# davxy/ark-vrf

Measured on AMD Instinct MI355X. Metric: thin_vrf_batch_verifications_per_sec, higher is better.
Workload: dtype u32x8 (256-bit prime-field Montgomery, integer)

## Files before the change

### ark_vrf_amd/csrc/curves.h

```cpp
#pragma once
#include <type_traits>
#include "fpn.h"
#include "te.h"
#include "fpu_te.h"
#include "fpu_g1.h"

#ifndef AVRF_TE_ACC_WAVES
#define AVRF_TE_ACC_WAVES 2
#endif
#ifndef AVRF_TE_ACC_MAX_WAVES
#define AVRF_TE_ACC_MAX_WAVES 2
#endif
#ifndef AVRF_G1_ACC_WAVES
#define AVRF_G1_ACC_WAVES 2
#endif
#ifndef AVRF_G1_RED_WAVES
#define AVRF_G1_RED_WAVES 1
#endif

#ifndef AVRF_G1_RED_INLINE
#define AVRF_G1_RED_INLINE 1
#endif

namespace avrf {

template <class CV> struct AccumSame {
  using acc_t = typename CV::acc_t; using base_t = typename CV::base_t;
  static AVRF_DI acc_t identity() { return CV::identity(); }
  static AVRF_DI acc_t madd(const acc_t &a, const base_t &q, bool neg) { return CV::madd(a, q, neg); }
  static AVRF_DI acc_t from_base(const base_t &q, bool neg) { return CV::from_base(q, neg); }
  static constexpr int PART_WORDS = CV::ACC_WORDS;
  static AVRF_DI void store_part(uint32_t *p, const acc_t &a) { CV::store_acc(p, a); }
  static AVRF_DI typename CV::acc_t load_part(const uint32_t *p) { return CV::load_acc(p); }
};
template <class S> struct AccumTeU {
  using acc_t = te_acc_u<S>; using base_t = te_pre;
  static AVRF_DI acc_t identity() { return teu_identity<S>(); }
  static AVRF_DI acc_t madd(const acc_t &a, const base_t &q, bool neg) { return teu_madd<S>(a, q, neg); }
  static AVRF_DI acc_t from_base(const base_t &q, bool neg) { return teu_from_pre<S>(q, neg); }
  static constexpr int PART_WORDS = TEU_PART_WORDS;
  static AVRF_DI void store_part(uint32_t *p, const acc_t &a) { teu_store_part<S>(p, a); }
  static AVRF_DI te_ext load_part(const uint32_t *p) { return teu_load_part<S>(p); }
};

template <class C> struct G1Curve;
template <class C> struct AccumG1U {
  using CV = G1Curve<C>; using Fq = typename C::Fq;
  using acc_t = g1_acc_u<C>; using base_t = typename CV::base_t;
  static AVRF_DI acc_t identity() { return g1u_identity<C>(); }
  static AVRF_DI acc_t madd(const acc_t &a, const base_t &q, bool neg) {
    return g1u_madd<C>(a, q.x.v, q.y.v, neg, [&]() {
      base_t t = q; if (neg) t.y = fn_neg<Fq>(t.y);
      const typename CV::acc_t r = CV::dbl_affine(t);
      return g1u_from_xyzz<C>(r.x.v, r.y.v, r.zz.v, r.zzz.v);
    });
  }
  static AVRF_DI acc_t from_base(const base_t &q, bool neg) { return g1u_from_affine<C>(q.x.v, q.y.v, neg); }
  static constexpr int PART_WORDS = G1UPart<C>::WORDS;
  static AVRF_DI void store_part(uint32_t *p, const acc_t &a) { g1u_store_part<C>(p, a); }
  static AVRF_DI typename CV::acc_t load_part(const uint32_t *p) {
    typename CV::acc_t r; g1u_load_part<C>(p, r.x.v, r.y.v, r.zz.v, r.zzz.v); return r;
  }
};

template <class S> struct TeCurve {
  using base_t = te_pre; using acc_t = te_ext; using suite = S;
#ifndef AVRF_NO_UNSAT
  using accum = typename std::conditional<!S::SW_NATIVE, AccumTeU<S>, AccumSame<TeCurve<S>>>::type;
#else
  using accum = AccumSame<TeCurve<S>>;
#endif
// ... 203 lines not shown
```

### ark_vrf_amd/csrc/fpu_te.h

```cpp
#pragma once
#include "fpu.h"
#include "te.h"

namespace avrf {

template <class S> struct te_acc_u {
  fuF<typename S::Fq> x, y, t, z;
  uint32_t neg;
};

template <class S> AVRF_DI te_acc_u<S> teu_identity() {
  using Fq = typename S::Fq;
  te_acc_u<S> r;
  r.x = fu_zero<UL<Fq>::L>(); r.t = r.x; r.y = fu_const<Fq>(UL<Fq>::ONE); r.z = r.y; r.neg = 0;
  return r;
}
template <class S> AVRF_DI te_acc_u<S> teu_from_pre(const te_pre &q, bool neg) {
  using Fq = typename S::Fq;
  te_acc_u<S> r;
  r.x = fu_slice<Fq, 0>(q.x.v); r.y = fu_slice<Fq, 0>(q.y.v);
  r.t = fu_mul<Fq>(r.x, fu_slice<Fq, UL<Fq>::SH>(q.y.v));
  r.z = fu_const<Fq>(UL<Fq>::ONE);
  r.neg = neg ? 0xffffffffu : 0u;
  return r;
}
template <class S> AVRF_DI te_acc_u<S> teu_madd(const te_acc_u<S> &p, const te_pre &q, bool neg) {
  using Fq = typename S::Fq;
  constexpr int SH = UL<Fq>::SH, L = UL<Fq>::L;
  const uint32_t e = neg ? 0xffffffffu : 0u;
  const int32_t flip = (int32_t)(p.neg ^ e);
  const fu<L> X1 = fu_cneg<L>(p.x, flip), T1 = fu_cneg<L>(p.t, flip);
  fp xy; add8(xy, q.x, q.y);
  const fu<L> A = fu_mul<Fq>(X1, fu_slice<Fq, SH>(q.x.v));
  const fu<L> B = fu_mul<Fq>(p.y, fu_slice<Fq, SH>(q.y.v));
  const fu<L> C = fu_mul<Fq>(T1, fu_slice<Fq, SH>(q.k.v));
  fu<L> E = fu_mul<Fq>(fu_add<L>(X1, p.y), fu_slice<Fq, SH>(xy.v));
  E = fu_sub<L>(fu_sub<L>(E, A), B);
  const fu<L> F = fu_sub<L>(p.z, C), G = fu_add<L>(p.z, C);
  fu<L> H;
  if (S::A_KIND == 1) {
    uint32_t h[L - 1];
#pragma unroll
    for (int i = 0; i < L - 1; i++) h[i] = (uint32_t)B.v[i] + 5u * (uint32_t)A.v[i];
    H = fu_carry_u<Fq>(h, B.v[L - 1] + 5 * A.v[L - 1]);
  } else if (S::A_KIND == 2) H = fu_carry<Fq>(fu_add<L>(B, A));
  else H = fu_sub<L>(B, A);
  te_acc_u<S> r;
  r.x = fu_mul<Fq>(E, F); r.y = fu_mul<Fq>(G, H); r.t = fu_mul<Fq>(E, H); r.z = fu_mul<Fq>(F, G);
  r.neg = e;
  return r;
}
template <class S> AVRF_DI te_ext teu_to_ext(const te_acc_u<S> &p) {
  using Fq = typename S::Fq;
  constexpr int L = UL<Fq>::L;
  te_ext r;
  fu_to_packed<Fq>(r.x.v, fu_cneg<L>(p.x, (int32_t)p.neg)); fu_to_packed<Fq>(r.y.v, p.y);
  fu_to_packed<Fq>(r.t.v, fu_cneg<L>(p.t, (int32_t)p.neg)); fu_to_packed<Fq>(r.z.v, p.z);
  return r;
}

template <class S> struct teu4 { fuF<typename S::Fq> x, y, t, z; };

template <class S> AVRF_DI teu4<S> teu4_identity() {
  using Fq = typename S::Fq;
  teu4<S> r; r.x = fu_zero<UL<Fq>::L>(); r.t = r.x; r.y = fu_const<Fq>(UL<Fq>::ONE); r.z = r.y; return r;
}
template <class S> AVRF_DI teu4<S> teu4_from_ext(const te_ext &e) {
  using Fq = typename S::Fq;
  teu4<S> r; r.x = fu_slice<Fq, 0>(e.x.v); r.y = fu_slice<Fq, 0>(e.y.v); r.t = fu_slice<Fq, 0>(e.t.v); r.z = fu_slice<Fq, 0>(e.z.v); return r;
}
template <class S> AVRF_DI te_ext teu4_to_ext(const teu4<S> &p) {
  using Fq = typename S::Fq;
  te_ext r; fu_to_packed<Fq>(r.x.v, p.x); fu_to_packed<Fq>(r.y.v, p.y); fu_to_packed<Fq>(r.t.v, p.t); fu_to_packed<Fq>(r.z.v, p.z); return r;
}
template <class S, int L> AVRF_DI fu<L> teu_h(const fu<L> &A, const fu<L> &B) {
  using Fq = typename S::Fq;
  if (S::A_KIND == 1) {
    uint32_t h[L - 1];
#pragma unroll
    for (int i = 0; i < L - 1; i++) h[i] = (uint32_t)B.v[i] + 5u * (uint32_t)A.v[i];
// ... 33 lines not shown
  const fu<L> C = fu_mul<Fq>(fu_mul<Fq>(p.t, fu_slice<Fq, SH>(e.t.v)), fu_slice<Fq, SH>(S::D));
  const fu<L> D = fu_mul<Fq>(p.z, fu_slice<Fq, SH>(e.z.v));
  fu<L> E = fu_mul<Fq>(fu_add<L>(p.x, p.y), fu_slice<Fq, SH>(xy.v));
  E = fu_sub<L>(fu_sub<L>(E, A), B);
  const fu<L> F = fu_sub<L>(D, C), G = fu_add<L>(D, C), H = teu_h<S, L>(A, B);
  teu4<S> r;
  r.x = fu_mul<Fq>(E, F); r.y = fu_mul<Fq>(G, H); r.t = fu_mul<Fq>(E, H); r.z = fu_mul<Fq>(F, G);
  return r;
}
template <class S> AVRF_DI teu4<S> teu4_madd_pre(const teu4<S> &p, const te_pre &q) {
  using Fq = typename S::Fq;
  constexpr int L = UL<Fq>::L, SH = UL<Fq>::SH;
  fp xy; add8(xy, q.x, q.y);
  const fu<L> A = fu_mul<Fq>(p.x, fu_slice<Fq, SH>(q.x.v)), B = fu_mul<Fq>(p.y, fu_slice<Fq, SH>(q.y.v));
  const fu<L> C = fu_mul<Fq>(p.t, fu_slice<Fq, SH>(q.k.v));
  fu<L> E = fu_mul<Fq>(fu_add<L>(p.x, p.y), fu_slice<Fq, SH>(xy.v));
  E = fu_sub<L>(fu_sub<L>(E, A), B);
  const fu<L> F = fu_sub<L>(p.z, C), G = fu_add<L>(p.z, C), H = teu_h<S, L>(A, B);
  teu4<S> r;
  r.x = fu_mul<Fq>(E, F); r.y = fu_mul<Fq>(G, H); r.t = fu_mul<Fq>(E, H); r.z = fu_mul<Fq>(F, G);
  return r;
}

constexpr int TEU_PART_WORDS = 40;
template <class S> AVRF_DI void teu_store_part(uint32_t *p, const te_acc_u<S> &a) {
  uint4 *d = reinterpret_cast<uint4 *>(p);
  const int32_t *x = a.x.v, *y = a.y.v, *t = a.t.v, *z = a.z.v;
  d[0] = make_uint4(x[0], x[1], x[2], x[3]); d[1] = make_uint4(x[4], x[5], x[6], x[7]);
  d[2] = make_uint4(x[8], y[0], y[1], y[2]); d[3] = make_uint4(y[3], y[4], y[5], y[6]);
  d[4] = make_uint4(y[7], y[8], t[0], t[1]); d[5] = make_uint4(t[2], t[3], t[4], t[5]);
  d[6] = make_uint4(t[6], t[7], t[8], z[0]); d[7] = make_uint4(z[1], z[2], z[3], z[4]);
  d[8] = make_uint4(z[5], z[6], z[7], z[8]); d[9] = make_uint4(a.neg, 0u, 0u, 0u);
}
template <class S> AVRF_DI fp teu_load_part_coord(const uint32_t *p, int j) {
  using Fq = typename S::Fq;
  constexpr int L = UL<Fq>::L;
  fu<L> v;
#pragma unroll
  for (int i = 0; i < L; i++) v.v[i] = (int32_t)p[j * L + i];
  const int32_t s = (j & 1) ? 0 : (int32_t)p[4 * L];
  fp r; fu_to_packed<Fq>(r.v, fu_cneg<L>(v, s));
  return r;
}
template <class S> AVRF_DI fuF<typename S::Fq> teu_load_part_coord_raw(const uint32_t *p, int j) {
  using Fq = typename S::Fq;
  constexpr int L = UL<Fq>::L;
  fu<L> v;
#pragma unroll
  for (int i = 0; i < L; i++) v.v[i] = (int32_t)p[j * L + i];
  const int32_t s = (j & 1) ? 0 : (int32_t)p[4 * L];
  return fu_cneg<L>(v, s);
}
template <class S> AVRF_DI te_ext teu_load_part(const uint32_t *p) {
  const uint4 *d = reinterpret_cast<const uint4 *>(p);
  uint32_t w[40];
#pragma unroll
  for (int i = 0; i < 10; i++) { const uint4 q = d[i]; w[4 * i] = q.x; w[4 * i + 1] = q.y; w[4 * i + 2] = q.z; w[4 * i + 3] = q.w; }
  te_acc_u<S> a;
#pragma unroll
  for (int i = 0; i < 9; i++) { a.x.v[i] = (int32_t)w[i]; a.y.v[i] = (int32_t)w[9 + i]; a.t.v[i] = (int32_t)w[18 + i]; a.z.v[i] = (int32_t)w[27 + i]; }
  a.neg = w[36];
  return teu_to_ext<S>(a);
}

}
```

### ark_vrf_amd/csrc/msm.h

```cpp
#pragma once
#include <hip/hip_runtime.h>
#include <stddef.h>
#include <stdint.h>
#include "host_te.h"

namespace avrf {

struct te_pre_raw { uint32_t w[24]; };
struct te_ext_raw { uint32_t w[32]; };

struct HipFailure { hipError_t err; const char *file; int line; };

template <bool PINNED> struct OwnedMem {
  void *p = nullptr; size_t cap = 0;
  OwnedMem() = default;
  explicit OwnedMem(size_t bytes) { ensure(bytes); }
  OwnedMem(const OwnedMem &) = delete;
  OwnedMem &operator=(const OwnedMem &) = delete;
  OwnedMem(OwnedMem &&o) noexcept : p(o.p), cap(o.cap) { o.p = nullptr; o.cap = 0; }
  OwnedMem &operator=(OwnedMem &&o) noexcept { if (this != &o) { (void)release(); p = o.p; cap = o.cap; o.p = nullptr; o.cap = 0; } return *this; }
  ~OwnedMem() { (void)release(); }
  hipError_t reset(size_t bytes) {
    if (hipError_t e = release()) return e;
    if (hipError_t e = PINNED ? hipHostMalloc(&p, bytes) : hipMalloc(&p, bytes)) { p = nullptr; return e; }
// ... 34 lines not shown
  MsmPlan plan = {0, 0, 0, 0}; int ret = 0;
  int wsum_lg = 4;
  size_t n = 0;
  bool armed = false;
  void ensure(size_t bytes);
  void disarm() { armed = false; }
  void release() { *this = MsmChain(); }
};

struct MsmWorkspace {
  DevMem keys;
  DevMem sorted;
  DevMem hist;
  DevMem cnts;
  DevMem offsets;
  DevMem win_tot;
  DevMem lane_base;
  DevMem heavy;
  DevMem plan_dev;
  DevMem buckets;
  DevMem rc;
  DevMem part;
  DevMem bits;
  MsmChain own;
  bool owns(const MsmChain &rec) const { return &rec == &own; }
  double accum_ms_total = 0; uint64_t accum_launches = 0; float accum_ms_last = 0;
  MsmPlan last_plan = {0, 0, 0, 0};
  void ensure(size_t n, const MsmPlan &p, size_t acc_bytes, size_t batch, size_t lanes_max, size_t part_bytes = 0);
  void release() { *this = MsmWorkspace(); }
};

int msm_te_device(int suite, const te_pre_raw *d_pre, const uint32_t *d_scalars, size_t n,
                  MsmWorkspace &ws, hipStream_t stream, HostExt *out);
int msm_te_enqueue(int suite, const te_pre_raw *d_pre, const uint32_t *d_scalars, size_t n, MsmWorkspace &ws, MsmChain &rec, hipStream_t stream);
int msm_te_finish(int suite, MsmWorkspace &ws, MsmChain &rec, hipStream_t stream, HostExt *out);
int msm_te_small_vectors(int suite, const te_pre_raw *d_pre, const uint32_t *d_scalars, size_t n, size_t n_vectors, MsmWorkspace &ws, hipStream_t stream,
                         HostExt *out);
bool msm_te_pending_supported(int suite);

int msm_g1_device(int curve, const uint32_t *d_bases, const uint32_t *d_scalars, size_t n, MsmWorkspace &ws, hipStream_t stream, uint8_t *out_xy,
                  size_t batch = 1, size_t scalar_stride = 0);
void build_g1_table(int curve, const uint32_t *d_bases, size_t n, int c, int nwin, uint32_t *d_table, hipStream_t stream);
int msm_g1_fixed_device(int curve, const uint32_t *d_table, int table_c, size_t table_stride, const uint32_t *d_scalars, size_t n,
                        size_t scalar_stride, MsmWorkspace &ws, hipStream_t stream, uint8_t *out_xy, size_t batch,
                        const uint32_t *d_base_idx = nullptr, int scalars_mont = 0);
struct G1DirectTable {
  uint32_t *d = nullptr;
  int curve = 0, c = 0, rows = 0;
  size_t n = 0;
  uint64_t off[32] = {};
  uint32_t mult[32] = {};
// ... 21 lines not shown
```

### ark_vrf_amd/csrc/msm.hip

```cpp
#include "msm.h"
#include "host_pool.h"
#include "curves.h"
#include "suite_dispatch.h"
#include "te_quad.h"
#include "host_g1.h"
#include <stdio.h>
#include <stdlib.h>
#include <string.h>
#include <mutex>
#include <vector>

namespace avrf {

#define HIP_CHECK(x) do { hipError_t e_ = (x); if (e_ != hipSuccess) throw HipFailure{e_, __FILE__, __LINE__}; } while (0)


template <class S>
__global__ void __launch_bounds__(256) k_pre_from_affine(const uint8_t *__restrict__ xy, uint32_t n, te_pre *__restrict__ out,
                                  uint32_t *__restrict__ flag, int check_curve, int mont_in) {
  using Fq = typename S::Fq;
  uint32_t i = blockIdx.x * blockDim.x + threadIdx.x;
  if (i >= n) return;
  fp x = fp_load_le(xy + 64 * (size_t)i), y = fp_load_le(xy + 64 * (size_t)i + 32);
  uint32_t f = 0;
// ... 7 lines not shown
void launch_pre_from_affine(int suite, const uint8_t *d_xy, size_t n, te_pre_raw *d_pre, uint32_t *d_flag,
                            int check_curve, hipStream_t stream, int mont_in) {
  if (!n) return;
  dim3 g((unsigned)((n + 255) / 256)), b(256);
  with_suite(suite, [&](auto tag) { using S = typename decltype(tag)::type;
    hipLaunchKernelGGL(k_pre_from_affine<S>, g, b, 0, stream, d_xy, (uint32_t)n, (te_pre *)d_pre, d_flag, check_curve, mont_in); });
}
template <class S>
__global__ void __launch_bounds__(256) k_scalars_from_mont(uint32_t *__restrict__ sc, uint32_t n, uint32_t *__restrict__ flag) {
  using Fr = typename S::Fr;
  uint32_t i = blockIdx.x * blockDim.x + threadIdx.x;
  if (i >= n) return;
  fp k = load_fp(sc + 8 * (size_t)i);
  if (ge_p<Fr>(k)) atomicOr(flag, 4u);
  store_fp(sc + 8 * (size_t)i, fp_from_mont<Fr>(k));
}
void launch_scalars_from_mont(int suite, uint32_t *d_scalars, size_t n, uint32_t *d_flag, hipStream_t stream) {
  if (!n) return;
  with_suite(suite, [&](auto tag) { using S = typename decltype(tag)::type;
    hipLaunchKernelGGL(k_scalars_from_mont<S>, dim3((unsigned)((n + 255) / 256)), dim3(256), 0, stream, d_scalars, (uint32_t)n, d_flag); });
}


__global__ void __launch_bounds__(256) k_digits(const uint32_t *__restrict__ scalars, uint32_t n, uint32_t stride, int c, int nwin, uint16_t *__restrict__ keys, int mont) {
  uint32_t i = blockIdx.x * blockDim.x + threadIdx.x;
  if (i >= n) return;
  const uint32_t bat = blockIdx.y;
  keys += (size_t)bat * nwin * n;
  uint32_t s[9];
  const uint4 *p = reinterpret_cast<const uint4 *>(scalars + 8 * ((size_t)bat * stride + i));
  uint4 a = p[0], b = p[1];
  s[0] = a.x; s[1] = a.y; s[2] = a.z; s[3] = a.w; s[4] = b.x; s[5] = b.y; s[6] = b.z; s[7] = b.w; s[8] = 0;
  if (mont) {
    fp v;
#pragma unroll
    for (int k = 0; k < 8; k++) v.v[k] = s[k];
    v = mont == 1 ? fp_from_mont<FqBandersnatch>(v) : fp_from_mont<FqBabyJubJub>(v);
#pragma unroll
    for (int k = 0; k < 8; k++) s[k] = v.v[k];
  }
  const uint32_t nb = 1u << (c - 1), mask = (1u << c) - 1;
  uint32_t carry = 0;
  for (int w = 0; w < nwin; w++) {
    int bit = w * c;
    uint32_t v = 0;
    if (bit < 256) {
      int li = bit >> 5, sh = bit & 31;
      uint64_t two = (uint64_t)s[li] | ((uint64_t)s[li + 1] << 32);
      v = (uint32_t)(two >> sh) & mask;
    }
    v += carry;
    uint32_t key;
    if (v > nb) { key = ((1u << c) - v) | 0x8000u; carry = 1; }
    else { key = v; carry = 0; }
    keys[(size_t)w * n + i] = (uint16_t)key;
  }
}


__global__ void __launch_bounds__(256)
k_hist(const uint16_t *__restrict__ keys, uint32_t n, uint32_t tile_len, int c, uint32_t *__restrict__ H) {
  extern __shared__ uint32_t lds[];
  const uint32_t nb = 1u << (c - 1), tile = blockIdx.x, w = blockIdx.y, ntiles = gridDim.x;
  for (uint32_t b = threadIdx.x; b < nb; b += blockDim.x) lds[b] = 0;
  __syncthreads();
  uint32_t lo = tile * tile_len, hi = lo + tile_len; if (hi > n) hi = n;
  const uint16_t *kw = keys + (size_t)w * n;
  for (uint32_t i = lo + threadIdx.x; i < hi; i += blockDim.x) {
    uint32_t b = kw[i] & 0x7fffu;
    if (b) atomicAdd(&lds[b - 1], 1u);
  }
  __syncthreads();
  uint32_t *out = H + ((size_t)w * ntiles + tile) * nb;
  for (uint32_t b = threadIdx.x; b < nb; b += blockDim.x) out[b] = lds[b];
}

__global__ void __launch_bounds__(256)
k_scan_tiles(uint32_t *__restrict__ H, uint32_t ntiles, int c, uint32_t *__restrict__ cnts) {
  const uint32_t nb = 1u << (c - 1), w = blockIdx.y, b = blockIdx.x * 256 + threadIdx.x;
// ... 95 lines not shown
    }
  }
}

template <class CV> __device__ __noinline__ void cv_add_nf(typename CV::acc_t *r, const typename CV::acc_t *a, const typename CV::acc_t *b) { *r = CV::add(*a, *b); }
template <class CV> __device__ __noinline__ void cv_dbl_nf(typename CV::acc_t *r, const typename CV::acc_t *a) { *r = CV::dbl(*a); }
template <class CV> AVRF_DI typename CV::acc_t cv_add(const typename CV::acc_t &a, const typename CV::acc_t &b) {
  if constexpr (CV::INLINE_REDUCE_OPS) return CV::add(a, b);
  else { typename CV::acc_t r; cv_add_nf<CV>(&r, &a, &b); return r; }
}
template <class CV> AVRF_DI typename CV::acc_t cv_dbl(const typename CV::acc_t &a) {
  if constexpr (CV::INLINE_REDUCE_OPS) return CV::dbl(a);
  else { typename CV::acc_t r; cv_dbl_nf<CV>(&r, &a); return r; }
}



template <class CV>
__global__ void __launch_bounds__(256, CV::MIN_WAVES)
k_accumulate(const uint32_t *__restrict__ bases, const uint32_t *__restrict__ sorted,
             const uint32_t *__restrict__ offs, const uint32_t *__restrict__ win_tot, const uint32_t *__restrict__ lane_base,
             const uint32_t *__restrict__ plan, uint32_t vwin, uint32_t nb, uint32_t n, uint32_t *__restrict__ part) {
  using AC = typename CV::accum;
  using acc_t = typename AC::acc_t; using base_t = typename CV::base_t;
  const uint32_t t = blockIdx.x * blockDim.x + threadIdx.x;
  const uint32_t per = plan[0];
  if (t >= plan[1]) return;
  uint32_t lo = 0, hi = vwin;
  while (hi - lo > 1) { uint32_t mid = (lo + hi) >> 1; if (lane_base[mid] <= t) lo = mid; else hi = mid; }
  const uint32_t v = lo;
  const uint32_t wbeg = v * n, wend = wbeg + win_tot[v];
  const uint32_t e0 = wbeg + (t - lane_base[v]) * per;
  uint32_t e1 = e0 + per; if (e1 > wend) e1 = wend;
  const uint32_t *ow = offs + (size_t)v * nb;
  lo = 0; hi = nb;
  while (hi - lo > 1) { uint32_t mid = (lo + hi) >> 1; if (ow[mid] <= e0) lo = mid; else hi = mid; }
  uint32_t b = lo;
  uint32_t nxt = (b + 1 < nb) ? ow[b + 1] : 0xffffffffu;
  const size_t slot0 = (size_t)t + (size_t)v * nb;
  acc_t acc;
  {
    extern __shared__ uint32_t acc_lds[];
    constexpr int BW = CV::BASE_WORDS, CH = BW / 4;
    uint32_t *wbuf = acc_lds + (threadIdx.x >> 6) * (2 * BW * 64);
    const uint32_t lane = threadIdx.x & 63;
    auto issue = [&](uint32_t ix, uint32_t slot) {
      const uint32_t *src = bases + (size_t)(ix & 0x7fffffffu) * BW;
#pragma unroll
      for (int c = 0; c < CH; c++)
        __builtin_amdgcn_global_load_lds((const __attribute__((address_space(1))) void *)(src + 4 * c),
                                         (__attribute__((address_space(3))) void *)(wbuf + slot * (BW * 64) + c * 256), 16, 0, 0);
    };
    auto fetch = [&](uint32_t slot) {
      uint32_t w[BW];
#pragma unroll
      for (int c = 0; c < CH; c++) {
        const uint4 v = *reinterpret_cast<const uint4 *>(wbuf + slot * (BW * 64) + c * 256 + lane * 4);
        w[4 * c] = v.x; w[4 * c + 1] = v.y; w[4 * c + 2] = v.z; w[4 * c + 3] = v.w;
      }
      return CV::base_from_words(w);
    };
    const uint32_t cnt = e1 - e0;
    if constexpr (!CV::PREFETCH) acc = AC::identity();
    uint32_t idx = cnt ? sorted[e0] : 0u;
    uint32_t idx1 = cnt > 1 ? sorted[e0 + 1] : 0u;
    if (cnt) issue(idx, 0);
    for (uint32_t k = 0; k < cnt; k++) {
      const uint32_t i = e0 + k, cidx = idx;
      asm volatile("s_waitcnt vmcnt(0) lgkmcnt(0)" ::: "memory");
      const base_t cur = fetch(k & 1);
      idx = idx1;
      if (k + 1 < cnt) issue(idx, (k + 1) & 1);
      if (k + 2 < cnt) idx1 = sorted[i + 2];
      if constexpr (CV::PREFETCH) {
        if (k == 0) { acc = AC::from_base(cur, (cidx & 0x80000000u) != 0); continue; }
      }
      if (i >= nxt) {
        AC::store_part(part + (slot0 + b) * AC::PART_WORDS, acc);
        acc = AC::identity();
        do { b++; nxt = (b + 1 < nb) ? ow[b + 1] : 0xffffffffu; } while (i >= nxt);
      }
      acc = AC::madd(acc, cur, (cidx & 0x80000000u) != 0);
    }
// ... 253 lines not shown
    HIP_CHECK(hipDeviceGetAttribute(&cus, hipDeviceAttributeMultiprocessorCount, dev));
    HIP_CHECK(hipOccupancyMaxActiveBlocksPerMultiprocessor(&blocks, k_accumulate<CV>, 256, 0));
    if (blocks < 1) blocks = 1;
    if (hipDeviceGetAttribute(&lds_cu, hipDeviceAttributeMaxSharedMemoryPerMultiprocessor, dev) != hipSuccess || lds_cu <= 0) { (void)hipGetLastError(); lds_cu = 0; }
    if (hipDeviceGetAttribute(&lds_blk, hipDeviceAttributeMaxSharedMemoryPerBlock, dev) != hipSuccess || lds_blk <= 0) { (void)hipGetLastError(); lds_blk = 64 * 1024; }
    {
      hipDeviceProp_t prop;
      if (hipGetDeviceProperties(&prop, dev) == hipSuccess && !strncmp(prop.gcnArchName, "gfx950", 6)) {
        if (lds_cu < 160 * 1024) lds_cu = 160 * 1024;
        if (lds_blk < 160 * 1024) lds_blk = 160 * 1024;
      } else (void)hipGetLastError();
    }
    int cap = CV::MAX_WAVES;
    if (msm_env().occ) cap = msm_env().occ;
    unsigned lds = 0;
    if (cap >= 1 && cap < blocks && lds_cu > 0) {
      const unsigned slice = (unsigned)(lds_cu / (cap + 1) + 1024);
      if ((size_t)slice * cap <= (size_t)lds_cu && slice <= (unsigned)lds_blk) {
        blocks = cap; lds = slice;
        if (lds > 48 * 1024) HIP_CHECK(hipFuncSetAttribute((const void *)k_accumulate<CV>, hipFuncAttributeMaxDynamicSharedMemorySize, (int)lds));
      }
    }
    {
      const unsigned need = 4u * 2u * CV::BASE_WORDS * 64u * 4u;
      if (lds < need) lds = need;
      if (lds > 48 * 1024) HIP_CHECK(hipFuncSetAttribute((const void *)k_accumulate<CV>, hipFuncAttributeMaxDynamicSharedMemorySize, (int)lds));
      int blk2 = 0;
      HIP_CHECK(hipOccupancyMaxActiveBlocksPerMultiprocessor(&blk2, k_accumulate<CV>, 256, lds));
      if (blk2 >= 1 && blk2 < blocks) blocks = blk2;
    }
    cache[dev] = AccShape{(size_t)cus * blocks * 256, lds};
  }
  return cache[dev];
}
template <class CV> static size_t accumulate_lanes() { return accumulate_shape<CV>().lanes; }

static bool msm_poison() { static const bool on = getenv("AVRF_MSM_POISON") != nullptr; return on; }
static void poison(void *p, size_t bytes, int which) {
  if (!msm_poison() || !p) return;
  if (const char *e = getenv("AVRF_MSM_POISON_SKIP")) { if (atoi(e) == which) return; }
  HIP_CHECK(hipMemset(p, 0xA5, bytes)); if (!getenv("AVRF_MSM_POISON_NOSYNC")) HIP_CHECK(hipDeviceSynchronize());
}
static void ws_buf(DevMem &m, size_t bytes, int which) {
  if (bytes <= m.cap) return;
  m.ensure(bytes);
  poison(m.p, bytes, which);
}

void MsmWorkspace::ensure(size_t n, const MsmPlan &p, size_t acc_bytes, size_t batch, size_t lanes_max, size_t part_bytes) {
  const size_t vwin = (size_t)p.nwin * batch;
  const size_t nbk = vwin * p.nb, nbits = vwin * p.c;
  const size_t need_n = vwin * n;
  const size_t ntiles = (n + tile_len_for(n, vwin) - 1) / tile_len_for(n, vwin);
  ws_buf(keys, need_n * 2 + 16, 1); ws_buf(sorted, need_n * 4 + 16, 2);
  ws_buf(hist, nbk * ntiles * 4 + 64, 3);
  ws_buf(cnts, nbk * 4, 4); ws_buf(offsets, nbk * 4, 5); ws_buf(heavy, nbk * 4, 6);
  ws_buf(win_tot, (vwin + 64) * 4, 7); ws_buf(lane_base, (vwin + 64) * 4, 8);
  plan_dev.ensure(64);
  ws_buf(buckets, nbk * acc_bytes, 9); ws_buf(rc, nbk * acc_bytes, 10);
  ws_buf(part, (lanes_max + nbk + 64) * (part_bytes ? part_bytes : acc_bytes) + 64, 11);
  ws_buf(bits, nbits * acc_bytes, 12); own.ensure(nbits * acc_bytes);
}

void MsmChain::ensure(size_t bytes) {
  if (!plan_host) { plan_host.ensure(64); plan_host.as()[0] = plan_host.as()[1] = 0; }
  if (!ev0) { HIP_CHECK(ev0.create()); HIP_CHECK(ev1.create()); }
  bits_host.ensure(bytes);
}

static void msm_collect(MsmWorkspace &ws, MsmChain &rec, hipStream_t stream) {
  if (ws.owns(rec)) { HIP_CHECK(hipStreamSynchronize(stream)); HIP_CHECK(hipGetLastError()); }
  HIP_CHECK(hipEventElapsedTime(&ws.accum_ms_last, rec.ev0, rec.ev1));
  rec.plan.lpb = (int)rec.plan_host.as()[0];
  ws.accum_ms_total += ws.accum_ms_last; ws.accum_launches++; ws.last_plan = rec.plan;
}

constexpr size_t MSM_TINY_TERMS = 2048, MSM_TINY_VECTORS = 32;
template <class CV>
__global__ void __launch_bounds__(256)
k_msm_tiny_bits(const uint32_t *__restrict__ bases, const uint32_t *__restrict__ scalars, uint32_t n, uint32_t stride, uint32_t *__restrict__ out) {
  extern __shared__ uint32_t lds[];
  const uint32_t p = blockIdx.x, v = blockIdx.y, t = threadIdx.x, T = blockDim.x, lane = t & 63, wv = t >> 6, nw = T >> 6;
  typename CV::acc_t acc = CV::identity();
  bool first = true;
// ... 47 lines not shown
                       (uint32_t)scalar_stride, ws.bits.as());
    HIP_CHECK(hipEventRecord(rec.ev1, stream));
    HIP_CHECK(hipMemcpyAsync(rec.bits_host.p, ws.bits.p, batch * nbits * acc_b, hipMemcpyDeviceToHost, stream));
    finish();
    return (int)nbits;
  }
  const size_t lanes_target = accumulate_lanes<CV>();
  size_t n = n_in;
  uint32_t remap_n = 0, remap_stride = 0;
  dim3 b256(256);
  int dig_nwin = p.nwin;
  if (table_c) {
    dig_nwin = (scalar_bits + 1 + table_c - 1) / table_c;
    p.c = table_c; p.nb = 1 << (table_c - 1); p.nwin = 1;
    n = n_in * (size_t)dig_nwin;
    remap_n = (uint32_t)n_in; remap_stride = (uint32_t)o.table_stride;
  }
  using RV = typename CV::red;
  const bool red = CV::FIXED_TABLE && table_c != 0;
  const size_t acc_bytes = (size_t)(red ? (int)RV::ACC_WORDS : (int)CV::ACC_WORDS) * 4;
  const uint32_t vwin = (uint32_t)(p.nwin * batch);
  const size_t lanes_max = lanes_target + vwin + 256;
  if ((size_t)vwin * n >= 0xffff0000ull) throw HipFailure{hipErrorInvalidValue, __FILE__, __LINE__};
  ws.ensure(n, p, acc_bytes, batch, lanes_max, (size_t)CV::accum::PART_WORDS * 4);
  const uint32_t nbk = vwin * p.nb;
  const uint32_t tile_len = tile_len_for(n, vwin), ntiles = (uint32_t)((n + tile_len - 1) / tile_len);
  const size_t lds_bytes = (size_t)p.nb * 4;
  hipLaunchKernelGGL(k_digits, dim3((unsigned)((n_in + 255) / 256), (unsigned)batch), b256, 0, stream, d_scalars, (uint32_t)n_in, (uint32_t)scalar_stride,
                     p.c, dig_nwin, ws.keys.as<uint16_t>(), scalars_mont);
  hipLaunchKernelGGL(k_hist, dim3(ntiles, vwin), b256, lds_bytes, stream, ws.keys.as<uint16_t>(), (uint32_t)n, tile_len, p.c, ws.hist.as());
  hipLaunchKernelGGL(k_scan_tiles, dim3((unsigned)((p.nb + 255) / 256), vwin), b256, 0, stream, ws.hist.as(), ntiles, p.c, ws.cnts.as());
  hipLaunchKernelGGL(k_scan_offs, dim3(vwin), dim3(1024), 0, stream, ws.cnts.as(), (uint32_t)n, p.c, ws.offsets.as(), ws.win_tot.as());
  hipLaunchKernelGGL(k_plan, dim3(1), dim3(1024), 0, stream, ws.win_tot.as(), vwin, (uint32_t)lanes_target, (uint32_t)msm_env().per_min,
                     ws.lane_base.as(), ws.plan_dev.as());
  hipLaunchKernelGGL(k_scatter, dim3(8u * ((vwin + 7u) / 8u) * ntiles), b256, lds_bytes, stream, ws.keys.as<uint16_t>(), (uint32_t)n, tile_len, p.c, ws.hist.as(),
                     ws.offsets.as(), ws.sorted.as(), remap_n, remap_stride, d_base_idx, ntiles, vwin);
  rec.ensure((size_t)vwin * 3 * acc_bytes);
  if (CV::ZERO_IS_IDENTITY) HIP_CHECK(hipMemsetAsync(ws.buckets.p, 0, (size_t)nbk * acc_bytes, stream));
  HIP_CHECK(hipEventRecord(rec.ev0, stream));
  hipLaunchKernelGGL(k_accumulate<CV>, dim3((unsigned)((lanes_max + 255) / 256)), b256, accumulate_shape<CV>().lds, stream, d_bases, ws.sorted.as(),
                     ws.offsets.as(), ws.win_tot.as(), ws.lane_base.as(), ws.plan_dev.as(), vwin, (uint32_t)p.nb, (uint32_t)n, ws.part.as());
  HIP_CHECK(hipEventRecord(rec.ev1, stream));
  auto bucket_sums = [&](auto tag) {
    using BV = typename decltype(tag)::type;
    hipLaunchKernelGGL(k_bucket_sum<BV>, dim3((nbk + 255) / 256), b256, 0, stream, ws.offsets.as(), ws.cnts.as(), ws.lane_base.as(), ws.plan_dev.as(), nbk,
                       (uint32_t)p.nb, (uint32_t)n, ws.part.as(), ws.buckets.as(), ws.heavy.as());
    hipLaunchKernelGGL(k_heavy_sum<BV>, dim3(nbk < 1024 ? nbk : 1024), b256, 4 * acc_bytes, stream, ws.offsets.as(), ws.cnts.as(), ws.lane_base.as(),
                       ws.plan_dev.as(), (uint32_t)p.nb, (uint32_t)n, ws.part.as(), ws.buckets.as(), ws.heavy.as());
  };
  if (red) bucket_sums(type_tag<RV>{}); else bucket_sums(type_tag<CV>{});
  HIP_CHECK(hipMemcpyAsync(rec.plan_host.p, ws.plan_dev.p, 8, hipMemcpyDeviceToHost, stream));
  rec.plan = p;
  if constexpr (CV::WINDOW_SUMS) if (batch == 1 && msm_env().window_sums) {
    const uint32_t nb = (uint32_t)p.nb;
    const uint32_t wpw = nb >= 256 ? 16u : 1u, m = nb >= 256 ? nb / 256 : (nb >= 16 ? nb / 16 : 1u);
    const uint32_t nwaves = vwin * wpw;
    hipLaunchKernelGGL(k_wsum_q1<typename CV::suite>, dim3((nwaves + 3) / 4), b256, 0, stream, ws.buckets.as(), nb, m, wpw, nwaves, ws.rc.as());
    hipLaunchKernelGGL(k_wsum_q2<typename CV::suite>, dim3(vwin), dim3(64), 0, stream, ws.rc.as(), wpw, ws.bits.as());
    HIP_CHECK(hipMemcpyAsync(rec.bits_host.p, ws.bits.p, (size_t)vwin * 3 * acc_bytes, hipMemcpyDeviceToHost, stream));
    rec.wsum_lg = 4; while ((1u << rec.wsum_lg) < 16 * m) rec.wsum_lg++;
    finish();
    return -(int)vwin;
  }
// ... 475 lines not shown
  uint32_t *o = idx + ((size_t)bat * n + i) * rows;
  const uint32_t ib = base_idx ? base_idx[(size_t)bat * n + i] : i;
  const uint32_t nb = 1u << (c - 1), mask = (1u << c) - 1;
  uint32_t carry = 0;
  for (uint32_t w = 0; w < rows; w++) {
    const int bit = (int)w * c;
    uint32_t v = 0;
    if (bit < 256) {
      const int li = bit >> 5, sh = bit & 31;
      const uint64_t two = (uint64_t)s[li] | ((uint64_t)(li + 1 < 9 ? s[li + 1] : 0u) << 32);
      v = (uint32_t)(two >> sh) & mask;
    }
    v += carry;
    uint32_t m, sign = 0;
    if (v > nb) { m = (1u << c) - v; sign = 0x80000000u; carry = 1; } else { m = v; carry = 0; }
    o[w] = (m == 0 || m > t.mult[w] || ib >= tn) ? DIRECT_ZERO : (uint32_t)(t.off[w] + (uint64_t)(m - 1) * tn + ib) | sign;
  }
}

template <class CV>
__global__ void __launch_bounds__(256, CV::MIN_WAVES)
k_accumulate_direct(const uint32_t *__restrict__ table, const uint32_t *__restrict__ idx, uint32_t E, uint32_t lpv, uint32_t per, uint32_t batch,
                    uint32_t *__restrict__ part) {
  using AC = typename CV::accum; using acc_t = typename AC::acc_t; using base_t = typename CV::base_t;
  const uint32_t t = blockIdx.x * blockDim.x + threadIdx.x;
  const uint32_t vec = t / lpv, r = t - vec * lpv;
  extern __shared__ uint32_t acc_lds[];
  constexpr int BW = CV::BASE_WORDS, CH = BW / 4;
  uint32_t *wbuf = acc_lds + (threadIdx.x >> 6) * (2 * BW * 64);
  const uint32_t lane = threadIdx.x & 63;
  const bool live = vec < batch;
  const size_t v0 = (size_t)(live ? vec : 0) * E;
  uint32_t cnt = 0; size_t e0 = v0;
  if (live && (uint64_t)r * per < E) { e0 = v0 + (size_t)r * per; cnt = (uint64_t)r * per + per <= E ? per : (uint32_t)(E - (uint64_t)r * per); }
  auto issue = [&](uint32_t ix, uint32_t slot) {
    const uint32_t *src = table + (size_t)(ix == DIRECT_ZERO ? 0u : (ix & 0x7fffffffu)) * BW;
#pragma unroll
    for (int c = 0; c < CH; c++)
      __builtin_amdgcn_global_load_lds((const __attribute__((address_space(1))) void *)(src + 4 * c),
                                       (__attribute__((address_space(3))) void *)(wbuf + slot * (BW * 64) + c * 256), 16, 0, 0);
  };
  auto fetch = [&](uint32_t slot) {
    uint32_t w[BW];
#pragma unroll
    for (int c = 0; c < CH; c++) {
      const uint4 v = *reinterpret_cast<const uint4 *>(wbuf + slot * (BW * 64) + c * 256 + lane * 4);
      w[4 * c] = v.x; w[4 * c + 1] = v.y; w[4 * c + 2] = v.z; w[4 * c + 3] = v.w;
// ... 80 lines not shown
```

Before: 131.6 million.

## Precompute signed unpacked-limb base table for TE bucket accumulation

The digit-decomposition kernel now also builds a per-call table holding each TE base in unpacked limb form, in both positive and negated versions, with x+y already added. The accumulate kernel gathers those entries by sign-encoded index, so the mixed add no longer needs per-step conditional negation, slicing or the x+y addition. Because negation now lives in the table, the accumulator drops its sign word and partial records shrink from 40 to 36 words. In exchange, each gathered entry is 28 words instead of the packed base, and the table must be written on every call.

```diff
diff --git a/ark_vrf_amd/csrc/curves.h b/ark_vrf_amd/csrc/curves.h
--- a/ark_vrf_amd/csrc/curves.h
+++ b/ark_vrf_amd/csrc/curves.h
@@ -26,6 +26,10 @@
 
 template <class CV> struct AccumSame {
   using acc_t = typename CV::acc_t; using base_t = typename CV::base_t;
+  static constexpr bool TABLE = false;
+  static constexpr int GATHER_WORDS = CV::BASE_WORDS, GATHER_STRIDE = CV::BASE_WORDS, TABLE_WORDS = 0;
+  static AVRF_DI uint32_t gather_index(uint32_t ix) { return ix & 0x7fffffffu; }
+  static AVRF_DI base_t base_from_words(const uint32_t (&w)[GATHER_WORDS]) { return CV::base_from_words(w); }
   static AVRF_DI acc_t identity() { return CV::identity(); }
   static AVRF_DI acc_t madd(const acc_t &a, const base_t &q, bool neg) { return CV::madd(a, q, neg); }
   static AVRF_DI acc_t from_base(const base_t &q, bool neg) { return CV::from_base(q, neg); }
@@ -34,10 +38,20 @@
   static AVRF_DI typename CV::acc_t load_part(const uint32_t *p) { return CV::load_acc(p); }
 };
 template <class S> struct AccumTeU {
-  using acc_t = te_acc_u<S>; using base_t = te_pre;
+  using acc_t = te_acc_u<S>; using base_t = te_limb<S>;
+  static constexpr bool TABLE = true;
+  static constexpr int GATHER_WORDS = TEU_GATHER_WORDS, GATHER_STRIDE = TEU_ENTRY_WORDS, TABLE_WORDS = 2 * TEU_ENTRY_WORDS;
+  static AVRF_DI uint32_t gather_index(uint32_t ix) { return (ix << 1) | (ix >> 31); }
+  static AVRF_DI base_t base_from_words(const uint32_t (&w)[GATHER_WORDS]) { return teu_limb_from_words<S>(w); }
+  static AVRF_DI void table_build(uint32_t *table, const uint32_t *bases, uint32_t i) {
+    const te_pre q = load_pre(reinterpret_cast<const te_pre *>(bases) + i);
+    uint32_t *e = table + (size_t)i * TABLE_WORDS;
+    teu_store_limb<S>(e, teu_limb_from_pre<S>(q, false));
+    teu_store_limb<S>(e + TEU_ENTRY_WORDS, teu_limb_from_pre<S>(q, true));
+  }
   static AVRF_DI acc_t identity() { return teu_identity<S>(); }
-  static AVRF_DI acc_t madd(const acc_t &a, const base_t &q, bool neg) { return teu_madd<S>(a, q, neg); }
-  static AVRF_DI acc_t from_base(const base_t &q, bool neg) { return teu_from_pre<S>(q, neg); }
+  static AVRF_DI acc_t madd(const acc_t &a, const base_t &q, bool) { return teu_madd<S>(a, q); }
+  static AVRF_DI acc_t from_base(const base_t &q, bool) { return teu_from_limb<S>(q); }
   static constexpr int PART_WORDS = TEU_PART_WORDS;
   static AVRF_DI void store_part(uint32_t *p, const acc_t &a) { teu_store_part<S>(p, a); }
   static AVRF_DI te_ext load_part(const uint32_t *p) { return teu_load_part<S>(p); }
@@ -47,6 +61,10 @@
 template <class C> struct AccumG1U {
   using CV = G1Curve<C>; using Fq = typename C::Fq;
   using acc_t = g1_acc_u<C>; using base_t = typename CV::base_t;
+  static constexpr bool TABLE = false;
+  static constexpr int GATHER_WORDS = 2 * Fq::N, GATHER_STRIDE = 2 * Fq::N, TABLE_WORDS = 0;
+  static AVRF_DI uint32_t gather_index(uint32_t ix) { return ix & 0x7fffffffu; }
+  static AVRF_DI base_t base_from_words(const uint32_t (&w)[GATHER_WORDS]) { return CV::base_from_words(w); }
   static AVRF_DI acc_t identity() { return g1u_identity<C>(); }
   static AVRF_DI acc_t madd(const acc_t &a, const base_t &q, bool neg) {
     return g1u_madd<C>(a, q.x.v, q.y.v, neg, [&]() {
diff --git a/ark_vrf_amd/csrc/fpu_te.h b/ark_vrf_amd/csrc/fpu_te.h
--- a/ark_vrf_amd/csrc/fpu_te.h
+++ b/ark_vrf_amd/csrc/fpu_te.h
@@ -4,37 +4,75 @@
 
 namespace avrf {
 
-template <class S> struct te_acc_u {
-  fuF<typename S::Fq> x, y, t, z;
-  uint32_t neg;
-};
+template <class S> struct te_limb { fuF<typename S::Fq> x, s, k; };
+constexpr int TEU_ENTRY_WORDS = 32, TEU_GATHER_WORDS = 28;
+
+template <class S> AVRF_DI te_limb<S> teu_limb_from_pre(const te_pre &q, bool neg) {
+  using Fq = typename S::Fq;
+  constexpr int SH = UL<Fq>::SH;
+  const fp x = neg ? fp_neg<Fq>(q.x) : q.x, k = neg ? fp_neg<Fq>(q.k) : q.k;
+  fp xy; add8(xy, x, q.y);
+  te_limb<S> r;
+  r.x = fu_slice<Fq, SH>(x.v); r.s = fu_slice<Fq, SH>(xy.v); r.k = fu_slice<Fq, SH>(k.v);
+  return r;
+}
+template <class S> AVRF_DI void teu_store_limb(uint32_t *p, const te_limb<S> &e) {
+  static_assert(UL<typename S::Fq>::L == 9, "entry layout: 3 x 9 limbs");
+  uint4 *d = reinterpret_cast<uint4 *>(p);
+  const int32_t *x = e.x.v, *s = e.s.v, *k = e.k.v;
+  d[0] = make_uint4(x[0], x[1], x[2], x[3]); d[1] = make_uint4(x[4], x[5], x[6], x[7]);
+  d[2] = make_uint4(x[8], s[0], s[1], s[2]); d[3] = make_uint4(s[3], s[4], s[5], s[6]);
+  d[4] = make_uint4(s[7], s[8], k[0], k[1]); d[5] = make_uint4(k[2], k[3], k[4], k[5]);
+  d[6] = make_uint4(k[6], k[7], k[8], 0u);
+}
+template <class S> AVRF_DI te_limb<S> teu_limb_from_words(const uint32_t (&w)[TEU_GATHER_WORDS]) {
+  te_limb<S> r;
+#pragma unroll
+  for (int i = 0; i < 9; i++) { r.x.v[i] = (int32_t)w[i]; r.s.v[i] = (int32_t)w[9 + i]; r.k.v[i] = (int32_t)w[18 + i]; }
+  return r;
+}
+template <class S> AVRF_DI te_limb<S> teu_load_limb(const uint32_t *p) {
+  const uint4 *d = reinterpret_cast<const uint4 *>(p);
+  uint32_t w[TEU_GATHER_WORDS];
+#pragma unroll
+  for (int i = 0; i < TEU_GATHER_WORDS / 4; i++) { const uint4 q = d[i]; w[4 * i] = q.x; w[4 * i + 1] = q.y; w[4 * i + 2] = q.z; w[4 * i + 3] = q.w; }
+  return teu_limb_from_words<S>(w);
+}
+
+template <class S> struct te_acc_u { fuF<typename S::Fq> x, y, t, z; };
 
 template <class S> AVRF_DI te_acc_u<S> teu_identity() {
   using Fq = typename S::Fq;
   te_acc_u<S> r;
-  r.x = fu_zero<UL<Fq>::L>(); r.t = r.x; r.y = fu_const<Fq>(UL<Fq>::ONE); r.z = r.y; r.neg = 0;
-  return r;
-}
-template <class S> AVRF_DI te_acc_u<S> teu_from_pre(const te_pre &q, bool neg) {
-  using Fq = typename S::Fq;
+  r.x = fu_zero<UL<Fq>::L>(); r.t = r.x; r.y = fu_const<Fq>(UL<Fq>::ONE); r.z = r.y;
+  return r;
+}
+template <class F> AVRF_DI fuF<F> fu_unshift(const fuF<F> &a) {
+  using U = UL<F>;
+  constexpr int L = U::L, SH = U::SH, W = U::W;
+  fuF<F> r;
+#pragma unroll
+  for (int i = 0; i < L - 1; i++) r.v[i] = (a.v[i] >> SH) + ((a.v[i + 1] & ((1 << SH) - 1)) << (W - SH));
+  r.v[L - 1] = a.v[L - 1] >> SH;
+  return r;
+}
+template <class S> AVRF_DI te_acc_u<S> teu_from_limb(const te_limb<S> &q) {
+  using Fq = typename S::Fq;
+  constexpr int L = UL<Fq>::L;
+  const fu<L> yb = fu_sub<L>(q.s, q.x);
   te_acc_u<S> r;
-  r.x = fu_slice<Fq, 0>(q.x.v); r.y = fu_slice<Fq, 0>(q.y.v);
-  r.t = fu_mul<Fq>(r.x, fu_slice<Fq, UL<Fq>::SH>(q.y.v));
+  r.x = fu_unshift<Fq>(q.x); r.y = fu_unshift<Fq>(yb);
+  r.t = fu_mul<Fq>(r.x, yb);
   r.z = fu_const<Fq>(UL<Fq>::ONE);
-  r.neg = neg ? 0xffffffffu : 0u;
-  return r;
-}
-template <class S> AVRF_DI te_acc_u<S> teu_madd(const te_acc_u<S> &p, const te_pre &q, bool neg) {
-  using Fq = typename S::Fq;
-  constexpr int SH = UL<Fq>::SH, L = UL<Fq>::L;
-  const uint32_t e = neg ? 0xffffffffu : 0u;
-  const int32_t flip = (int32_t)(p.neg ^ e);
-  const fu<L> X1 = fu_cneg<L>(p.x, flip), T1 = fu_cneg<L>(p.t, flip);
-  fp xy; add8(xy, q.x, q.y);
-  const fu<L> A = fu_mul<Fq>(X1, fu_slice<Fq, SH>(q.x.v));
-  const fu<L> B = fu_mul<Fq>(p.y, fu_slice<Fq, SH>(q.y.v));
-  const fu<L> C = fu_mul<Fq>(T1, fu_slice<Fq, SH>(q.k.v));
-  fu<L> E = fu_mul<Fq>(fu_add<L>(X1, p.y), fu_slice<Fq, SH>(xy.v));
+  return r;
+}
+template <class S> AVRF_DI te_acc_u<S> teu_madd(const te_acc_u<S> &p, const te_limb<S> &q) {
+  using Fq = typename S::Fq;
+  constexpr int L = UL<Fq>::L;
+  const fu<L> A = fu_mul<Fq>(p.x, q.x);
+  const fu<L> B = fu_mul<Fq>(p.y, fu_sub<L>(q.s, q.x));
+  const fu<L> C = fu_mul<Fq>(p.t, q.k);
+  fu<L> E = fu_mul<Fq>(fu_add<L>(p.x, p.y), q.s);
   E = fu_sub<L>(fu_sub<L>(E, A), B);
   const fu<L> F = fu_sub<L>(p.z, C), G = fu_add<L>(p.z, C);
   fu<L> H;
@@ -47,15 +85,12 @@
   else H = fu_sub<L>(B, A);
   te_acc_u<S> r;
   r.x = fu_mul<Fq>(E, F); r.y = fu_mul<Fq>(G, H); r.t = fu_mul<Fq>(E, H); r.z = fu_mul<Fq>(F, G);
-  r.neg = e;
   return r;
 }
 template <class S> AVRF_DI te_ext teu_to_ext(const te_acc_u<S> &p) {
   using Fq = typename S::Fq;
-  constexpr int L = UL<Fq>::L;
   te_ext r;
-  fu_to_packed<Fq>(r.x.v, fu_cneg<L>(p.x, (int32_t)p.neg)); fu_to_packed<Fq>(r.y.v, p.y);
-  fu_to_packed<Fq>(r.t.v, fu_cneg<L>(p.t, (int32_t)p.neg)); fu_to_packed<Fq>(r.z.v, p.z);
+  fu_to_packed<Fq>(r.x.v, p.x); fu_to_packed<Fq>(r.y.v, p.y); fu_to_packed<Fq>(r.t.v, p.t); fu_to_packed<Fq>(r.z.v, p.z);
   return r;
 }
 
@@ -135,7 +170,7 @@
   return r;
 }
 
-constexpr int TEU_PART_WORDS = 40;
+constexpr int TEU_PART_WORDS = 36;
 template <class S> AVRF_DI void teu_store_part(uint32_t *p, const te_acc_u<S> &a) {
   uint4 *d = reinterpret_cast<uint4 *>(p);
   const int32_t *x = a.x.v, *y = a.y.v, *t = a.t.v, *z = a.z.v;
@@ -143,36 +178,28 @@
   d[2] = make_uint4(x[8], y[0], y[1], y[2]); d[3] = make_uint4(y[3], y[4], y[5], y[6]);
   d[4] = make_uint4(y[7], y[8], t[0], t[1]); d[5] = make_uint4(t[2], t[3], t[4], t[5]);
   d[6] = make_uint4(t[6], t[7], t[8], z[0]); d[7] = make_uint4(z[1], z[2], z[3], z[4]);
-  d[8] = make_uint4(z[5], z[6], z[7], z[8]); d[9] = make_uint4(a.neg, 0u, 0u, 0u);
+  d[8] = make_uint4(z[5], z[6], z[7], z[8]);
+}
+template <class S> AVRF_DI fuF<typename S::Fq> teu_load_part_coord_raw(const uint32_t *p, int j) {
+  using Fq = typename S::Fq;
+  constexpr int L = UL<Fq>::L;
+  fu<L> v;
+#pragma unroll
+  for (int i = 0; i < L; i++) v.v[i] = (int32_t)p[j * L + i];
+  return v;
 }
 template <class S> AVRF_DI fp teu_load_part_coord(const uint32_t *p, int j) {
-  using Fq = typename S::Fq;
-  constexpr int L = UL<Fq>::L;
-  fu<L> v;
-#pragma unroll
-  for (int i = 0; i < L; i++) v.v[i] = (int32_t)p[j * L + i];
-  const int32_t s = (j & 1) ? 0 : (int32_t)p[4 * L];
-  fp r; fu_to_packed<Fq>(r.v, fu_cneg<L>(v, s));
-  return r;
-}
-template <class S> AVRF_DI fuF<typename S::Fq> teu_load_part_coord_raw(const uint32_t *p, int j) {
-  using Fq = typename S::Fq;
-  constexpr int L = UL<Fq>::L;
-  fu<L> v;
-#pragma unroll
-  for (int i = 0; i < L; i++) v.v[i] = (int32_t)p[j * L + i];
-  const int32_t s = (j & 1) ? 0 : (int32_t)p[4 * L];
-  return fu_cneg<L>(v, s);
+  fp r; fu_to_packed<typename S::Fq>(r.v, teu_load_part_coord_raw<S>(p, j));
+  return r;
 }
 template <class S> AVRF_DI te_ext teu_load_part(const uint32_t *p) {
   const uint4 *d = reinterpret_cast<const uint4 *>(p);
-  uint32_t w[40];
-#pragma unroll
-  for (int i = 0; i < 10; i++) { const uint4 q = d[i]; w[4 * i] = q.x; w[4 * i + 1] = q.y; w[4 * i + 2] = q.z; w[4 * i + 3] = q.w; }
+  uint32_t w[TEU_PART_WORDS];
+#pragma unroll
+  for (int i = 0; i < TEU_PART_WORDS / 4; i++) { const uint4 q = d[i]; w[4 * i] = q.x; w[4 * i + 1] = q.y; w[4 * i + 2] = q.z; w[4 * i + 3] = q.w; }
   te_acc_u<S> a;
 #pragma unroll
   for (int i = 0; i < 9; i++) { a.x.v[i] = (int32_t)w[i]; a.y.v[i] = (int32_t)w[9 + i]; a.t.v[i] = (int32_t)w[18 + i]; a.z.v[i] = (int32_t)w[27 + i]; }
-  a.neg = w[36];
   return teu_to_ext<S>(a);
 }
 
diff --git a/ark_vrf_amd/csrc/msm.h b/ark_vrf_amd/csrc/msm.h
--- a/ark_vrf_amd/csrc/msm.h
+++ b/ark_vrf_amd/csrc/msm.h
@@ -80,11 +80,13 @@
   DevMem rc;
   DevMem part;
   DevMem bits;
+  DevMem table;
   MsmChain own;
   bool owns(const MsmChain &rec) const { return &rec == &own; }
   double accum_ms_total = 0; uint64_t accum_launches = 0; float accum_ms_last = 0;
   MsmPlan last_plan = {0, 0, 0, 0};
-  void ensure(size_t n, const MsmPlan &p, size_t acc_bytes, size_t batch, size_t lanes_max, size_t part_bytes = 0);
+  void ensure(size_t n, const MsmPlan &p, size_t acc_bytes, size_t batch, size_t lanes_max, size_t part_bytes = 0,
+              size_t table_bytes = 0);
   void release() { *this = MsmWorkspace(); }
 };
 
diff --git a/ark_vrf_amd/csrc/msm.hip b/ark_vrf_amd/csrc/msm.hip
--- a/ark_vrf_amd/csrc/msm.hip
+++ b/ark_vrf_amd/csrc/msm.hip
@@ -53,10 +53,8 @@
 }
 
 
-__global__ void __launch_bounds__(256) k_digits(const uint32_t *__restrict__ scalars, uint32_t n, uint32_t stride, int c, int nwin, uint16_t *__restrict__ keys, int mont) {
-  uint32_t i = blockIdx.x * blockDim.x + threadIdx.x;
-  if (i >= n) return;
-  const uint32_t bat = blockIdx.y;
+AVRF_DI void digits_lane(const uint32_t *__restrict__ scalars, uint32_t n, uint32_t stride, int c, int nwin, uint16_t *__restrict__ keys, int mont, uint32_t i,
+                         uint32_t bat) {
   keys += (size_t)bat * nwin * n;
   uint32_t s[9];
   const uint4 *p = reinterpret_cast<const uint4 *>(scalars + 8 * ((size_t)bat * stride + i));
@@ -86,6 +84,19 @@
     else { key = v; carry = 0; }
     keys[(size_t)w * n + i] = (uint16_t)key;
   }
+}
+__global__ void __launch_bounds__(256) k_digits(const uint32_t *__restrict__ scalars, uint32_t n, uint32_t stride, int c, int nwin, uint16_t *__restrict__ keys, int mont) {
+  uint32_t i = blockIdx.x * blockDim.x + threadIdx.x;
+  if (i >= n) return;
+  digits_lane(scalars, n, stride, c, nwin, keys, mont, i, blockIdx.y);
+}
+template <class AC>
+__global__ void __launch_bounds__(256) k_digits_table(const uint32_t *__restrict__ scalars, uint32_t n, uint32_t stride, int c, int nwin, uint16_t *__restrict__ keys, int mont,
+                                                      const uint32_t *__restrict__ bases, uint32_t *__restrict__ table) {
+  uint32_t i = blockIdx.x * blockDim.x + threadIdx.x;
+  if (i >= n) return;
+  if (blockIdx.y == 0) AC::table_build(table, bases, i);
+  digits_lane(scalars, n, stride, c, nwin, keys, mont, i, blockIdx.y);
 }
 
 
@@ -227,7 +238,7 @@
              const uint32_t *__restrict__ offs, const uint32_t *__restrict__ win_tot, const uint32_t *__restrict__ lane_base,
              const uint32_t *__restrict__ plan, uint32_t vwin, uint32_t nb, uint32_t n, uint32_t *__restrict__ part) {
   using AC = typename CV::accum;
-  using acc_t = typename AC::acc_t; using base_t = typename CV::base_t;
+  using acc_t = typename AC::acc_t; using base_t = typename AC::base_t;
   const uint32_t t = blockIdx.x * blockDim.x + threadIdx.x;
   const uint32_t per = plan[0];
   if (t >= plan[1]) return;
@@ -246,11 +257,11 @@
   acc_t acc;
   {
     extern __shared__ uint32_t acc_lds[];
-    constexpr int BW = CV::BASE_WORDS, CH = BW / 4;
+    constexpr int BW = AC::GATHER_WORDS, CH = BW / 4;
     uint32_t *wbuf = acc_lds + (threadIdx.x >> 6) * (2 * BW * 64);
     const uint32_t lane = threadIdx.x & 63;
     auto issue = [&](uint32_t ix, uint32_t slot) {
-      const uint32_t *src = bases + (size_t)(ix & 0x7fffffffu) * BW;
+      const uint32_t *src = bases + (size_t)AC::gather_index(ix) * AC::GATHER_STRIDE;
 #pragma unroll
       for (int c = 0; c < CH; c++)
         __builtin_amdgcn_global_load_lds((const __attribute__((address_space(1))) void *)(src + 4 * c),
@@ -263,7 +274,7 @@
         const uint4 v = *reinterpret_cast<const uint4 *>(wbuf + slot * (BW * 64) + c * 256 + lane * 4);
         w[4 * c] = v.x; w[4 * c + 1] = v.y; w[4 * c + 2] = v.z; w[4 * c + 3] = v.w;
       }
-      return CV::base_from_words(w);
+      return AC::base_from_words(w);
     };
     const uint32_t cnt = e1 - e0;
     if constexpr (!CV::PREFETCH) acc = AC::identity();
@@ -563,7 +574,7 @@
       }
     }
     {
-      const unsigned need = 4u * 2u * CV::BASE_WORDS * 64u * 4u;
+      const unsigned need = 4u * 2u * CV::accum::GATHER_WORDS * 64u * 4u;
       if (lds < need) lds = need;
       if (lds > 48 * 1024) HIP_CHECK(hipFuncSetAttribute((const void *)k_accumulate<CV>, hipFuncAttributeMaxDynamicSharedMemorySize, (int)lds));
       int blk2 = 0;
@@ -588,7 +599,7 @@
   poison(m.p, bytes, which);
 }
 
-void MsmWorkspace::ensure(size_t n, const MsmPlan &p, size_t acc_bytes, size_t batch, size_t lanes_max, size_t part_bytes) {
+void MsmWorkspace::ensure(size_t n, const MsmPlan &p, size_t acc_bytes, size_t batch, size_t lanes_max, size_t part_bytes, size_t table_bytes) {
   const size_t vwin = (size_t)p.nwin * batch;
   const size_t nbk = vwin * p.nb, nbits = vwin * p.c;
   const size_t need_n = vwin * n;
@@ -601,6 +612,7 @@
   ws_buf(buckets, nbk * acc_bytes, 9); ws_buf(rc, nbk * acc_bytes, 10);
   ws_buf(part, (lanes_max + nbk + 64) * (part_bytes ? part_bytes : acc_bytes) + 64, 11);
   ws_buf(bits, nbits * acc_bytes, 12); own.ensure(nbits * acc_bytes);
+  if (table_bytes) ws_buf(table, table_bytes, 13);
 }
 
 void MsmChain::ensure(size_t bytes) {
@@ -694,12 +706,20 @@
   const uint32_t vwin = (uint32_t)(p.nwin * batch);
   const size_t lanes_max = lanes_target + vwin + 256;
   if ((size_t)vwin * n >= 0xffff0000ull) throw HipFailure{hipErrorInvalidValue, __FILE__, __LINE__};
-  ws.ensure(n, p, acc_bytes, batch, lanes_max, (size_t)CV::accum::PART_WORDS * 4);
+  using AC = typename CV::accum;
+  ws.ensure(n, p, acc_bytes, batch, lanes_max, (size_t)AC::PART_WORDS * 4, AC::TABLE ? n_in * (size_t)AC::TABLE_WORDS * 4 : 0);
   const uint32_t nbk = vwin * p.nb;
   const uint32_t tile_len = tile_len_for(n, vwin), ntiles = (uint32_t)((n + tile_len - 1) / tile_len);
   const size_t lds_bytes = (size_t)p.nb * 4;
-  hipLaunchKernelGGL(k_digits, dim3((unsigned)((n_in + 255) / 256), (unsigned)batch), b256, 0, stream, d_scalars, (uint32_t)n_in, (uint32_t)scalar_stride,
-                     p.c, dig_nwin, ws.keys.as<uint16_t>(), scalars_mont);
+  const uint32_t *gather = d_bases;
+  if constexpr (AC::TABLE) {
+    if (table_c || d_base_idx) throw HipFailure{hipErrorInvalidValue, __FILE__, __LINE__};
+    gather = ws.table.as();
+    hipLaunchKernelGGL(k_digits_table<AC>, dim3((unsigned)((n_in + 255) / 256), (unsigned)batch), b256, 0, stream, d_scalars, (uint32_t)n_in, (uint32_t)scalar_stride,
+                       p.c, dig_nwin, ws.keys.as<uint16_t>(), scalars_mont, d_bases, ws.table.as());
+  } else
+    hipLaunchKernelGGL(k_digits, dim3((unsigned)((n_in + 255) / 256), (unsigned)batch), b256, 0, stream, d_scalars, (uint32_t)n_in, (uint32_t)scalar_stride,
+                       p.c, dig_nwin, ws.keys.as<uint16_t>(), scalars_mont);
   hipLaunchKernelGGL(k_hist, dim3(ntiles, vwin), b256, lds_bytes, stream, ws.keys.as<uint16_t>(), (uint32_t)n, tile_len, p.c, ws.hist.as());
   hipLaunchKernelGGL(k_scan_tiles, dim3((unsigned)((p.nb + 255) / 256), vwin), b256, 0, stream, ws.hist.as(), ntiles, p.c, ws.cnts.as());
   hipLaunchKernelGGL(k_scan_offs, dim3(vwin), dim3(1024), 0, stream, ws.cnts.as(), (uint32_t)n, p.c, ws.offsets.as(), ws.win_tot.as());
@@ -710,7 +730,7 @@
   rec.ensure((size_t)vwin * 3 * acc_bytes);
   if (CV::ZERO_IS_IDENTITY) HIP_CHECK(hipMemsetAsync(ws.buckets.p, 0, (size_t)nbk * acc_bytes, stream));
   HIP_CHECK(hipEventRecord(rec.ev0, stream));
-  hipLaunchKernelGGL(k_accumulate<CV>, dim3((unsigned)((lanes_max + 255) / 256)), b256, accumulate_shape<CV>().lds, stream, d_bases, ws.sorted.as(),
+  hipLaunchKernelGGL(k_accumulate<CV>, dim3((unsigned)((lanes_max + 255) / 256)), b256, accumulate_shape<CV>().lds, stream, gather, ws.sorted.as(),
                      ws.offsets.as(), ws.win_tot.as(), ws.lane_base.as(), ws.plan_dev.as(), vwin, (uint32_t)p.nb, (uint32_t)n, ws.part.as());
   HIP_CHECK(hipEventRecord(rec.ev1, stream));
   auto bucket_sums = [&](auto tag) {
@@ -1232,7 +1252,7 @@
 __global__ void __launch_bounds__(256, CV::MIN_WAVES)
 k_accumulate_direct(const uint32_t *__restrict__ table, const uint32_t *__restrict__ idx, uint32_t E, uint32_t lpv, uint32_t per, uint32_t batch,
                     uint32_t *__restrict__ part) {
-  using AC = typename CV::accum; using acc_t = typename AC::acc_t; using base_t = typename CV::base_t;
+  using AC = typename CV::accum; using acc_t = typename AC::acc_t; using base_t = typename AC::base_t;
   const uint32_t t = blockIdx.x * blockDim.x + threadIdx.x;
   const uint32_t vec = t / lpv, r = t - vec * lpv;
   extern __shared__ uint32_t acc_lds[];
```

After: 131.3 million. No clear change (-0.2%).
